# musevlt/muse-psfr

Measured on AMD Instinct MI355X. Metric: PSFs/sec (row x lambda) on 512^2 grid, 35 lambda, higher is better.
Workload: dtype f64 PSD->structure function, per-lambda OTF f32 -> split-fp16 MFMA (fp32 accumulate), f64 fit

## Files before the change

### muse_psfr_amd/csrc/fit_common.h

```cpp
#pragma once
#include <hip/hip_runtime.h>
#include "device_common.h"

namespace mpsfr {
namespace {

template <int CTRL, int ROW_MASK>
__device__ __forceinline__ float dpp_term(float v) {
    return __builtin_bit_cast(float, __builtin_amdgcn_update_dpp(
                                         0, __builtin_bit_cast(int, v), CTRL, ROW_MASK, 0xf, false));
}
template <int CTRL, int ROW_MASK>
__device__ __forceinline__ double dpp_term(double v) {
    const long long b = __builtin_bit_cast(long long, v);
    const unsigned lo = (unsigned)__builtin_amdgcn_update_dpp(0, (int)(b & 0xffffffffll), CTRL,
                                                              ROW_MASK, 0xf, false);
    const unsigned hi = (unsigned)__builtin_amdgcn_update_dpp(0, (int)(b >> 32), CTRL, ROW_MASK,
                                                              0xf, false);
    return __builtin_bit_cast(double, ((long long)hi << 32) | (long long)lo);
}
__device__ __forceinline__ float lane63(float x) {
    return __builtin_bit_cast(float, __builtin_amdgcn_readlane(__builtin_bit_cast(int, x), 63));
}
__device__ __forceinline__ double lane63(double x) {
    const long long b = __builtin_bit_cast(long long, x);
    const unsigned lo = (unsigned)__builtin_amdgcn_readlane((int)(b & 0xffffffffll), 63);
    const unsigned hi = (unsigned)__builtin_amdgcn_readlane((int)(b >> 32), 63);
    return __builtin_bit_cast(double, ((long long)hi << 32) | (long long)lo);
}
template <typename T>
__device__ __forceinline__ T wave_total(T v) {
    v += dpp_term<0xB1, 0xf>(v);
    v += dpp_term<0x4E, 0xf>(v);
    v += dpp_term<0x141, 0xf>(v);
    v += dpp_term<0x140, 0xf>(v);
    v += dpp_term<0x142, 0xf>(v);
    v += dpp_term<0x143, 0xf>(v);
    return lane63(v);
}

template <typename RE>
__device__ __forceinline__ RE fit_log(RE x);
template <>
__device__ __forceinline__ float fit_log<float>(float x) { return __logf(x); }
template <>
__device__ __forceinline__ double fit_log<double>(double x) { return log(x); }
template <typename RE>
__device__ __forceinline__ RE fit_exp(RE x);
template <>
__device__ __forceinline__ float fit_exp<float>(float x) { return __expf(x); }
template <>
__device__ __forceinline__ double fit_exp<double>(double x) { return exp(x); }

template <typename S>
__device__ __forceinline__ S fit_rcp(S x);
template <>
__device__ __forceinline__ float fit_rcp<float>(float x) { return __builtin_amdgcn_rcpf(x); }
template <>
__device__ __forceinline__ double fit_rcp<double>(double x) { return 1.0 / x; }
template <typename S>
__device__ __forceinline__ S fit_rsqrt(S x);
template <>
__device__ __forceinline__ float fit_rsqrt<float>(float x) { return __builtin_amdgcn_rsqf(x); }
template <>
__device__ __forceinline__ double fit_rsqrt<double>(double x) {
    double y = __builtin_amdgcn_rsq(x);
    const double h = 0.5 * x;
    y = fma(y, fma(-h * y, y, 0.5), y);
    y = fma(y, fma(-h * y, y, 0.5), y);
    return y;
}

__device__ __forceinline__ double lean_exp(double z) {
    z = fmax(z, -700.0);
    const double k = rint(z * 1.4426950408889634074);
    double r = fma(-k, 6.93147180369123816490e-01, z);
    r = fma(-k, 1.90821492927058770002e-10, r);
    double p = 1.0 / 3628800.0;
    p = fma(p, r, 1.0 / 362880.0);
    p = fma(p, r, 1.0 / 40320.0);
    p = fma(p, r, 1.0 / 5040.0);
    p = fma(p, r, 1.0 / 720.0);
    p = fma(p, r, 1.0 / 120.0);
    p = fma(p, r, 1.0 / 24.0);
    p = fma(p, r, 1.0 / 6.0);
    p = fma(p, r, 0.5);
    p = fma(p, r, 1.0);
    p = fma(p, r, 1.0);
    return ldexp(p, (int)k);
}
__device__ __forceinline__ double lean_log(double x) {
    const double l0 = (double)(__builtin_amdgcn_logf((float)x) * 0.69314718f);
    const double d = fma(x, lean_exp(-l0), -1.0);
    return l0 + d * fma(d, fma(d, 1.0 / 3.0, -0.5), 1.0);
}

template <typename RE>
__device__ __forceinline__ RE fit_exp2m1(RE eta);
template <>
__device__ __forceinline__ float fit_exp2m1<float>(float eta) {
    return __builtin_amdgcn_exp2f(eta) - 1.0f;
}
template <>
__device__ __forceinline__ double fit_exp2m1<double>(double eta) {
    return lean_exp(0.69314718055994530942 * eta) - 1.0;
}

template <typename RE>
__device__ __forceinline__ RE fit_log2(RE x);
template <>
__device__ __forceinline__ float fit_log2<float>(float x) { return __builtin_amdgcn_logf(x); }
template <>
__device__ __forceinline__ double fit_log2<double>(double x) { return log(x) * 1.4426950408889634074; }
template <typename RE>
__device__ __forceinline__ RE fit_exp2(RE x);
template <>
__device__ __forceinline__ float fit_exp2<float>(float x) { return __builtin_amdgcn_exp2f(x); }
template <>
__device__ __forceinline__ double fit_exp2<double>(double x) { return exp(x * 0.69314718055994530942); }

__device__ __forceinline__ double sgpr(double x) {
    const long long b = __builtin_bit_cast(long long, x);
    const unsigned lo = (unsigned)__builtin_amdgcn_readfirstlane((int)(b & 0xffffffffll));
    const unsigned hi = (unsigned)__builtin_amdgcn_readfirstlane((int)(b >> 32));
    return __builtin_bit_cast(double, ((long long)hi << 32) | (long long)lo);
}


constexpr double kFitIllCond = 100.0;
constexpr double kFitMaxE = 0.95;
#ifndef MPSFR_FIT_MAXIT
#define MPSFR_FIT_MAXIT 200
#endif
constexpr int kFitMaxIt = MPSFR_FIT_MAXIT;
constexpr double kFitMu0 = 1.0e-2, kFitMuMax = 1.0e15;

template <typename T, int NP>
struct FitNormEq {
    T a[NP * (NP + 1) / 2];
    T g[NP];
    T chi2;
};

template <int NP>
__host__ __device__ constexpr int fit_diag(int k) { return k * NP - k * (k - 1) / 2; }

template <int NP, typename S, typename T, bool ROW_FIRST = false>
__device__ __forceinline__ bool fit_chol(const FitNormEq<T, NP>& ne, S mu, S L[NP][NP], S Li[NP], S id[NP]) {
    bool ok = true;
#pragma unroll
    for (int i = 0; i < NP; ++i) {
        const S d = (S)ne.a[fit_diag<NP>(i)];
        ok = ok && (d > (S)0);
        id[i] = fit_rsqrt<S>(d);
    }
    {
        int k = 0;
#pragma unroll
        for (int i = 0; i < NP; ++i)
#pragma unroll
            for (int j = i; j < NP; ++j) {
                L[j][i] = ROW_FIRST ? (S)ne.a[k] * id[j] * id[i] : (S)ne.a[k] * id[i] * id[j];
                ++k;
            }
    }
#pragma unroll
    for (int j = 0; j < NP; ++j) {
        S s = (S)1 + mu;
#pragma unroll
        for (int q = 0; q < j; ++q) s -= L[j][q] * L[j][q];
        ok = ok && (s > (S)0);
        Li[j] = fit_rsqrt<S>(s);
        L[j][j] = s * Li[j];
#pragma unroll
        for (int i = j + 1; i < NP; ++i) {
            S t = L[i][j];
#pragma unroll
            for (int q = 0; q < j; ++q) t -= L[i][q] * L[j][q];
            L[i][j] = t * Li[j];
        }
    }
    return ok;
}

template <int NP, typename S, typename X>
__device__ __forceinline__ void fit_chol_solve(const S L[NP][NP], const S Li[NP], const S id[NP], const S b[NP],
                                               X* x) {
    S y[NP], z[NP];
#pragma unroll
    for (int i = 0; i < NP; ++i) {
        S t = b[i] * id[i];
#pragma unroll
        for (int q = 0; q < i; ++q) t -= L[i][q] * y[q];
        y[i] = t * Li[i];
    }
#pragma unroll
    for (int i = NP - 1; i >= 0; --i) {
        S t = y[i];
#pragma unroll
        for (int q = i + 1; q < NP; ++q) t -= L[q][i] * z[q];
        z[i] = t * Li[i];
    }
#pragma unroll
    for (int i = 0; i < NP; ++i) x[i] = (X)(z[i] * id[i]);
}

template <int NP, typename S, typename T, bool ROW_FIRST = false>
__device__ __forceinline__ bool fit_lm_solve(const FitNormEq<T, NP>& ne, S mu, S* x) {
    S L[NP][NP], Li[NP], id[NP], b[NP];
    if (!fit_chol<NP, S, T, ROW_FIRST>(ne, mu, L, Li, id)) return false;
#pragma unroll
    for (int i = 0; i < NP; ++i) b[i] = -(S)ne.g[i];
    fit_chol_solve<NP, S, S>(L, Li, id, b, x);
    return true;
}

template <int NP, typename T, bool ROW_FIRST = false>
__device__ __forceinline__ bool fit_spd_inverse(const FitNormEq<T, NP>& ne, double cov[NP][NP]) {
    T L[NP][NP], Li[NP], id[NP];
    if (!fit_chol<NP, T, T, ROW_FIRST>(ne, (T)0, L, Li, id)) return false;
#pragma unroll
    for (int c = 0; c < NP; ++c) {
        T b[NP];
        double x[NP];
#pragma unroll
        for (int k = 0; k < NP; ++k) b[k] = (k == c) ? (T)1 : (T)0;
        fit_chol_solve<NP, T, double>(L, Li, id, b, x);
#pragma unroll
        for (int k = 0; k < NP; ++k) cov[k][c] = x[k];
    }
    return true;
}

template <typename RE, bool ELL>
struct MoffatPar {
    RE I, p0, q0, n, gK, A, B, C, e1g2, e2g2, w2, nsq2, dKn;
    __device__ __forceinline__ MoffatPar(const RE* v, int ieta) {
        I = v[0]; p0 = v[1]; q0 = v[2];
        n = fit_rcp<RE>(v[ieta]);
        const RE s_ = fit_exp2m1<RE>(v[ieta]);
        const RE iw = fit_rcp<RE>(v[3]);
        const RE K = (RE)4 * s_ * iw * iw;
        if constexpr (ELL) {
            const RE e1 = v[4], e2 = v[5];
            const RE g2 = fit_rcp<RE>((RE)1 - e1 * e1 - e2 * e2);
            const RE g = fit_rsqrt<RE>((RE)1 - e1 * e1 - e2 * e2);
            gK = g * K;
            A = gK * ((RE)1 - e1); B = gK * e2; C = gK * ((RE)1 + e1);
            e1g2 = e1 * g2; e2g2 = e2 * g2;
        } else {
            gK = K; A = K; B = (RE)0; C = K; e1g2 = (RE)0; e2g2 = (RE)0;
        }
        w2 = (RE)2 * iw;
        nsq2 = n * n * (RE)0.69314718055994530942;
        dKn = (s_ + (RE)1) * (RE)0.69314718055994530942 * fit_rcp<RE>(s_);
    }
};

__device__ __forceinline__ bool fit_moment_start(float ms1, float ms2, float best, int rm, float* eta0, double* fw0) {
    const float bf = best, r2 = ((float)rm + 0.5f) * ((float)rm + 0.5f);
    if (!(rm >= 6 && ms1 > 0.f && best > 0.f)) return false;
    float t1 = 1.f, t2 = 1.f, nn = 2.5f, a2 = 1.f;
#pragma unroll 1
    for (int k = 0; k < 6; ++k) {
        float rho = (ms2 * t1) * __builtin_amdgcn_rcpf(bf * ms1 * t2);
        rho = fminf(fmaxf(rho, 0.05f), 0.47f);
        nn = (1.f - rho) * __builtin_amdgcn_rcpf(1.f - 2.f * rho);
        nn = fminf(fmaxf(nn, 1.1f), 15.f);
        a2 = ms1 * (nn - 1.f) * __builtin_amdgcn_rcpf(t1 * bf * 3.14159265f);
        const float lx = __builtin_amdgcn_logf(1.f + r2 * __builtin_amdgcn_rcpf(a2));
        t1 = 1.f - __builtin_amdgcn_exp2f((1.f - nn) * lx);
        t2 = 1.f - __builtin_amdgcn_exp2f((1.f - 2.f * nn) * lx);
    }
    *eta0 = __builtin_amdgcn_rcpf(nn);
    const float w = 2.f * __builtin_amdgcn_sqrtf(a2 * (__builtin_amdgcn_exp2f(*eta0) - 1.f));
    if (w == w) *fw0 = fmin(fmax((double)w, 1.5), (double)NS);
    return true;
}

}
}
```

### muse_psfr_amd/csrc/stamps.hip

```cpp
#include "device_common.h"
#include "conv_frames.h"
#include "fit_common.h"

namespace mpsfr {

namespace {

template <typename R>
__global__ void __launch_bounds__(256)
k_moffat_kernels(const double* __restrict__ gam, const double* __restrict__ alp,
                 R* __restrict__ out) {
    __shared__ double part[4];
    __shared__ double tot;
    const int k = blockIdx.x;
    const double g2 = gam[k] * gam[k], al = alp[k];
    double vals[(KS * KS + 255) / 256];
    double s = 0.0;
#pragma unroll
    for (int m = 0; m < (KS * KS + 255) / 256; ++m) {
        const int e = threadIdx.x + m * 256;
        double v = 0.0;
        if (e < KS * KS) {
            const int dy = e / KS - KS / 2, dx = e % KS - KS / 2;
            const double x1 = 1.0 + (double)(dx * dx + dy * dy) / g2;
            v = al == 2.0 ? 1.0 / (x1 * x1) : pow(x1, -al);
        }
        vals[m] = v;
        s += v;
    }
    s = wave_sum(s);
    if ((threadIdx.x & 63) == 0) part[threadIdx.x >> 6] = s;
    __syncthreads();
    if (threadIdx.x == 0) tot = (part[0] + part[1]) + (part[2] + part[3]);
    __syncthreads();
    const double inv = 1.0 / tot;
#pragma unroll
    for (int m = 0; m < (KS * KS + 255) / 256; ++m) {
        const int e = threadIdx.x + m * 256;
        if (e < KS * KS) out[(size_t)k * KS * KS + e] = (R)(vals[m] * inv);
    }
}

template <typename R>
struct Vec4;
template <>
struct Vec4<float> { using type = float4; };
template <>
struct Vec4<double> { using type = double4; };

template <typename R>
__global__ void __launch_bounds__(256)
k_conv(int nl, int tdiv, const R* __restrict__ pre, const R* __restrict__ ktt,
       const R* __restrict__ kmuse, double* __restrict__ fin) {
    constexpr int PH = NS + KS - 1;
    constexpr int PW = 84;
    constexpr int HK = KS / 2;
    constexpr int SW = 8;
    constexpr int LW = SW + KS - 1;
    constexpr int NSTRIP = NS * NS / SW;
    using V4 = typename Vec4<R>::type;
    extern __shared__ __align__(32) unsigned char smem[];
    R* img = reinterpret_cast<R*>(smem);
    const int l = blockIdx.x, task = blockIdx.y;
    const R* src = pre + ((size_t)task * nl + l) * NS * NS;
    for (int e = threadIdx.x; e < PH * PW; e += 256) {
        const int P = e / PW - HK, Q = e % PW - HK;
        img[e] = (P >= 0 && P < NS && Q >= 0 && Q < NS) ? (R)src[P * NS + Q] : (R)0;
    }
    static_assert(NSTRIP == 200 && NS == 40, "strip map assumes 40x40 stamps");
    const int wv = threadIdx.x >> 6, ln = threadIdx.x & 63;
    const bool active = ln < 50;
    const int i = 10 * wv + (active ? ln % 10 : 0), j0 = (active ? ln / 10 : 0) * SW;
    double acc[SW];
    for (int pass = 0; pass < 2; ++pass) {
        const R* __restrict__ kg = pass == 0 ? ktt + (size_t)(task / tdiv) * KS * KS
                                             : kmuse + (size_t)l * KS * KS;
        __syncthreads();
#pragma unroll
        for (int o = 0; o < SW; ++o) acc[o] = 0.0;
        for (int a = 0; a <= HK; ++a) {
            const V4* r1 = reinterpret_cast<const V4*>(
                __builtin_assume_aligned(img + (i - a + 2 * HK) * PW + j0, sizeof(V4)));
            const V4* r2 = reinterpret_cast<const V4*>(
                __builtin_assume_aligned(img + (i + a) * PW + j0, sizeof(V4)));
            R sv[LW];
#pragma unroll
            for (int c = 0; c < LW / 4; ++c) {
                const V4 q = r1[c];
                sv[4 * c] = q.x; sv[4 * c + 1] = q.y; sv[4 * c + 2] = q.z; sv[4 * c + 3] = q.w;
            }
            if (a < HK) {
#pragma unroll
                for (int c = 0; c < LW / 4; ++c) {
                    const V4 q = r2[c];
                    sv[4 * c] += q.x; sv[4 * c + 1] += q.y; sv[4 * c + 2] += q.z; sv[4 * c + 3] += q.w;
                }
            }
            R part[SW];
#pragma unroll
            for (int o = 0; o < SW; ++o) part[o] = (R)0;
            const R* __restrict__ krow = kg + a * KS;
#pragma unroll
            for (int b = 0; b < KS; ++b) {
                const R kv = krow[b];
#pragma unroll
                for (int o = 0; o < SW; ++o) part[o] += kv * sv[o - b + 2 * HK];
            }
#pragma unroll
            for (int o = 0; o < SW; ++o) acc[o] += (double)part[o];
        }
        __syncthreads();
        if (pass == 0 && active) {
#pragma unroll
            for (int o = 0; o < SW; ++o) img[(i + HK) * PW + j0 + HK + o] = (R)acc[o];
        }
    }
    if (active) {
        double* out = fin + ((size_t)task * nl + l) * NS * NS + i * NS + j0;
#pragma unroll
        for (int o = 0; o < SW; ++o) out[o] = acc[o];
    }
}

template <typename R, typename TF>
#ifndef MPSFR_CONV_WAVES
#define MPSFR_CONV_WAVES 4
#endif
__global__ void __launch_bounds__(256) __attribute__((amdgpu_waves_per_eu(sizeof(R) == 4 ? MPSFR_CONV_WAVES : 2)))
k_conv_fft(int nl, int tdiv, const R* __restrict__ pre, const cx<R>* __restrict__ khat_tt,
           const cx<R>* __restrict__ khat_muse, TF* __restrict__ fin) {
    extern __shared__ __align__(16) unsigned char conv_smem[];
    cx<R> (*F)[CFP] = reinterpret_cast<cx<R> (*)[CFP]>(conv_smem);
    cx<R> (*bufs)[CFB] = reinterpret_cast<cx<R> (*)[CFB]>(conv_smem + sizeof(cx<R>) * CF * CFP);
    const int l = blockIdx.x, task = blockIdx.y;
    const int slot = threadIdx.x >> 3, t = threadIdx.x & 7;
    Tw64<R> tw;
    tw.init(t);
    const R* src = pre + ((size_t)task * nl + l) * NS * NS;
    cx<R>* buf = bufs[slot];
    cx<R> x[8];
#pragma unroll
    for (int e = 0; e < 8; ++e) {
        const int c = t + 8 * e;
        const bool in = c < NS && slot < NS / 2;
        x[e] = {in ? src[2 * slot * NS + c] : (R)0, in ? src[(2 * slot + 1) * NS + c] : (R)0};
    }
    for (int pass = 0; pass < 2; ++pass) {
        const cx<R>* __restrict__ kh = pass == 0 ? khat_tt + (size_t)(task / tdiv) * (CFH + 1) * CF
                                                     : khat_muse + (size_t)l * (CFH + 1) * CF;
        cx<R> khv[8], khn[8];
#pragma unroll
        for (int e = 0; e < 8; ++e) {
            khv[e] = kh[slot * CF + t + 8 * e];
            khn[e] = slot == 0 ? kh[CFH * CF + t + 8 * e] : cx<R>{(R)0, (R)0};
        }
        __syncthreads();
        if (slot < NS / 2) cf_rows_forward(x, F, buf, tw, slot, t);
        __syncthreads();
        {
            cx<R> y[8];
            if (slot == 0) {
                const cx<R>* res = cf_col_forward(F, NS, buf, tw, slot, t);
#pragma unroll
                for (int e = 0; e < 8; ++e) {
                    cx<R> a0, a32;
                    cf_split0(res, t + 8 * e, a0, a32);
                    const cx<R> b0 = cmul(a0, khv[e]), b32 = cmul(a32, khn[e]);
                    y[e] = conjf<R>(cx<R>{b0.x - b32.y, b0.y + b32.x});
                }
                fft_sync<true>();
            } else {
                cx<R> xin[8], v[8];
#pragma unroll
                for (int e = 0; e < 8; ++e) {
                    const int r = t + 8 * e;
                    xin[e] = r < NS ? F[r][slot] : cx<R>{(R)0, (R)0};
                }
                fft_forward_regs_lastreg<R, CF, true>(xin, buf, buf, tw.w, t, v);
#pragma unroll
                for (int e = 0; e < 8; ++e) y[e] = conjf<R>(cmul(v[e], khv[e]));
                fft_sync<true>();
            }
            cx<R> r2[8];
            fft_forward_regs_lastreg<R, CF, true>(y, buf, buf, tw.w, t, r2);
#pragma unroll
            for (int e = 0; e < 8; ++e) {
                const int r = t + 8 * e;
                if (r >= KS / 2 && r < KS / 2 + NS) F[r][slot] = conjf<R>(r2[e]);
            }
        }
        __syncthreads();
        if (slot < NS / 2) {
            const int ra = KS / 2 + 2 * slot, rb = ra + 1;
            cx<R> z[8];
#pragma unroll
            for (int e = 0; e < 8; ++e) {
                const int k = t + 8 * e;
                const int kk = k <= CFH ? k : CF - k;
                cx<R> a, b;
                if (kk == 0) {
                    a = {F[ra][0].x, (R)0};
                    b = {F[rb][0].x, (R)0};
                } else if (kk == CFH) {
                    a = {F[ra][0].y, (R)0};
                    b = {F[rb][0].y, (R)0};
                } else {
                    a = F[ra][kk];
                    b = F[rb][kk];
                    if (k > CFH) { a = conjf<R>(a); b = conjf<R>(b); }
                }
                z[e] = {a.x - b.y, -(a.y + b.x)};
            }
            if (pass == 1) {
                cx<R> v[8];
                fft_forward_regs_lastreg<R, CF, true>(z, buf, buf, tw.w, t, v);
                TF* out = fin + ((size_t)task * nl + l) * NS * NS;
#pragma unroll
                for (int e = 0; e < 8; ++e) {
                    const int c = t + 8 * e;
                    if (c >= KS / 2 && c < KS / 2 + NS) {
                        const int i = 2 * slot, j = c - KS / 2;
                        out[i * NS + j] = (TF)v[e].x;
                        out[(i + 1) * NS + j] = (TF)(-v[e].y);
                    }
                }
            } else {
                const cx<R>* res = fft_forward_regs<R, CF, true>(z, buf, buf, tw.w, t);
#pragma unroll
                for (int e = 0; e < 8; ++e) {
                    const int c = t + 8 * e;
                    const cx<R> v = res[lds_out<CF, 8>(c < NS ? c + KS / 2 : 0)];
                    x[e] = c < NS ? cx<R>{v.x, -v.y} : cx<R>{(R)0, (R)0};
                }
            }
        }
    }
}

template <typename R>
__global__ void __launch_bounds__(256)
k_khat(const double* __restrict__ gam, const double* __restrict__ alp, cx<R>* __restrict__ khat) {
    extern __shared__ __align__(16) unsigned char conv_smem[];
    khat_body<R>(gam, alp, khat, conv_smem, (int)blockIdx.x);
}



typedef float f32x2 __attribute__((ext_vector_type(2)));

template <typename RE>
struct NormAcc {
    RE a[15], g[5], chi2;
    __device__ __forceinline__ void zero() {
#pragma unroll
        for (int k = 0; k < 15; ++k) a[k] = (RE)0;
#pragma unroll
        for (int k = 0; k < 5; ++k) g[k] = (RE)0;
        chi2 = (RE)0;
    }
    __device__ __forceinline__ void add(const RE* J, RE r) {
        chi2 += r * r;
        int k = 0;
#pragma unroll
        for (int x = 0; x < 5; ++x) {
            g[x] += J[x] * r;
#pragma unroll
            for (int y = x; y < 5; ++y) a[k++] += J[x] * J[y];
        }
    }
    template <typename F>
    __device__ __forceinline__ void totals(FitNormEq<RE, 5>& ne, F total) const {
        ne.chi2 = total(chi2);
#pragma unroll
        for (int k = 0; k < 15; ++k) ne.a[k] = total(a[k]);
#pragma unroll
        for (int k = 0; k < 5; ++k) ne.g[k] = total(g[k]);
    }
};
template <>
struct NormAcc<float> {
    f32x2 r0a, r0b, r0c;
    f32x2 r1b, r1c;
    f32x2 r2b, r2c;
    f32x2 r3c, r4c;
    float a11, a33, chi2;
    __device__ __forceinline__ void zero() {
        const f32x2 z = {0.f, 0.f};
        r0a = r0b = r0c = r1b = r1c = r2b = r2c = r3c = r4c = z;
        a11 = a33 = chi2 = 0.f;
    }
    __device__ __forceinline__ void add(const float* J, float r) {
        const f32x2 p01 = {J[0], J[1]}, p23 = {J[2], J[3]}, p4r = {J[4], r};
        const f32x2 s0 = {J[0], J[0]}, s1 = {J[1], J[1]}, s2 = {J[2], J[2]}, s3 = {J[3], J[3]},
                    s4 = {J[4], J[4]};
        r0a += s0 * p01; r0b += s0 * p23; r0c += s0 * p4r;
        r1b += s1 * p23; r1c += s1 * p4r;
        r2b += s2 * p23; r2c += s2 * p4r;
        r3c += s3 * p4r;
        r4c += s4 * p4r;
        a11 += J[1] * J[1];
        a33 += J[3] * J[3];
        chi2 += r * r;
    }
    template <typename F>
    __device__ __forceinline__ void totals(FitNormEq<float, 5>& ne, F total) const {
        ne.chi2 = total(chi2);
        const float a[15] = {r0a.x, r0a.y, r0b.x, r0b.y, r0c.x, a11, r1b.x, r1b.y, r1c.x,
                             r2b.x, r2b.y, r2c.x, a33, r3c.x, r4c.x};
        const float g[5] = {r0c.y, r1c.y, r2c.y, r3c.y, r4c.y};
#pragma unroll
        for (int k = 0; k < 15; ++k) ne.a[k] = total(a[k]);
#pragma unroll
        for (int k = 0; k < 5; ++k) ne.g[k] = total(g[k]);
    }
};

template <typename RE>
__device__ __forceinline__ void moffat_accumulate(const RE* pix, int lane, const RE* v,
                                                  FitNormEq<RE, 5>& ne) {
    constexpr int NPX = NS * NS / 64;
    NormAcc<RE> acc;
    acc.zero();
    const RE n = fit_rcp<RE>(v[4]);
    const RE s_ = fit_exp2m1<RE>(v[4]);
    const RE i3 = fit_rcp<RE>(v[3]);
    const RE K = (RE)4 * s_ * i3 * i3;
    const RE dKn = (s_ + (RE)1) * (RE)0.69314718055994530942 * fit_rcp<RE>(s_);
    const RE I = v[0], p0 = v[1], q0 = v[2];
    const RE nsq2 = n * n * (RE)0.69314718055994530942;
    const RE c12 = (RE)2 * n * K, c3 = c12 * i3, c4 = n * K * dKn;
    const RE lrf = (RE)(lane >> 3) - p0, lcf = (RE)(lane & 7) - q0;
    const RE* pl = pix + (lane >> 3) * NS + (lane & 7);
    static_assert(NPX == 25 && NS == 40, "5 x 5 blocks of 8 x 8 pixels");
#pragma unroll 1
    for (int mo = 0; mo < 5; ++mo) {
        const RE dp = (RE)(8 * mo) + lrf, dp2 = dp * dp;
#pragma unroll
        for (int mi = 0; mi < 5; ++mi) {
        const RE dq = (RE)(8 * mi) + lcf;
        const RE u = dq * dq + dp2;
        const RE gg = (RE)1 + u * K;
        const RE lg2 = fit_log2<RE>(gg);
        const RE e = fit_exp2<RE>(-n * lg2);
        const RE mo_ = I * e;
        const RE r = mo_ - pl[mo * 8 * NS + mi * 8];
        const RE t = mo_ * fit_rcp<RE>(gg);
        const RE tu = t * u, tc = t * c12;
        RE J[5];
        J[0] = e;
        J[1] = tc * dp;
        J[2] = tc * dq;
        J[3] = tu * c3;
        J[4] = mo_ * (nsq2 * lg2) - tu * c4;
        acc.add(J, r);
        }
    }
    acc.totals(ne, [](RE x) { return wave_total(x); });
}

#ifndef MPSFR_FIT_PAIRS
#define MPSFR_FIT_PAIRS 1
#endif
__device__ __forceinline__ void moffat_accumulate_pairs(const float* pix, int lane, const float* v,
                                                        FitNormEq<float, 5>& ne) {
    f32x2 A[15], G[5], C = {0.f, 0.f};
#pragma unroll
    for (int k = 0; k < 15; ++k) A[k] = f32x2{0.f, 0.f};
#pragma unroll
    for (int k = 0; k < 5; ++k) G[k] = f32x2{0.f, 0.f};
    const float n = fit_rcp<float>(v[4]);
    const float s_ = fit_exp2m1<float>(v[4]);
    const float i3 = fit_rcp<float>(v[3]);
    const float K = 4.f * s_ * i3 * i3;
    const float dKn = (s_ + 1.f) * 0.69314718f * fit_rcp<float>(s_);
    const float I = v[0], p0 = v[1], q0 = v[2];
    const float nsq2 = n * n * 0.69314718f;
    const float c12 = 2.f * n * K, c3 = c12 * i3, c4 = n * K * dKn;
    const f32x2 K2 = {K, K}, I2 = {I, I}, nn2 = {-n, -n}, nsq22 = {nsq2, nsq2}, c122 = {c12, c12},
                c32 = {c3, c3}, c42 = {c4, c4}, one2 = {1.f, 1.f};
    const float lrf = (float)(lane >> 3) - p0, lcf = (float)(lane & 7) - q0;
    const float* pl = pix + (lane >> 3) * NS + (lane & 7);
    auto pair = [&](f32x2 u, f32x2 dpv, f32x2 dqv, f32x2 px, bool last) {
        const f32x2 gg = u * K2 + one2;
        const f32x2 lg2 = {fit_log2<float>(gg.x), fit_log2<float>(gg.y)};
        const f32x2 arg = lg2 * nn2;
        f32x2 e = {fit_exp2<float>(arg.x), fit_exp2<float>(arg.y)};
        if (last) e.y = 0.f;
        const f32x2 m = e * I2;
        const f32x2 r = m - px;
        const f32x2 rg = {fit_rcp<float>(gg.x), fit_rcp<float>(gg.y)};
        const f32x2 t = m * rg;
        const f32x2 tu = t * u, tc = t * c122;
        f32x2 J[5];
        J[0] = e;
        J[1] = tc * dpv;
        J[2] = tc * dqv;
        J[3] = tu * c32;
        J[4] = m * (lg2 * nsq22) - tu * c42;
        C += r * r;
        int k = 0;
#pragma unroll
        for (int x = 0; x < 5; ++x) {
            G[x] += J[x] * r;
#pragma unroll
            for (int y = x; y < 5; ++y) A[k++] += J[x] * J[y];
        }
    };
    const f32x2 dqa = {lcf, 8.f + lcf}, dqb = {16.f + lcf, 24.f + lcf};
    const f32x2 dqa2 = dqa * dqa, dqb2 = dqb * dqb;
    const float dq4 = 32.f + lcf, dq4s = dq4 * dq4;
#pragma unroll 1
    for (int mo = 0; mo < 5; ++mo) {
        const float dp = (float)(8 * mo) + lrf, dp2 = dp * dp;
        const f32x2 dpv = {dp, dp}, dp2v = {dp2, dp2};
        const float* row = pl + mo * 8 * NS;
        pair(dqa2 + dp2v, dpv, dqa, f32x2{row[0], row[8]}, false);
        pair(dqb2 + dp2v, dpv, dqb, f32x2{row[16], row[24]}, false);
    }
    {
        const f32x2 dq4v = {dq4, dq4}, dq4sv = {dq4s, dq4s};
        const f32x2 dpa = {lrf, 8.f + lrf}, dpb = {16.f + lrf, 24.f + lrf};
        const float dp4 = 32.f + lrf;
        pair(dpa * dpa + dq4sv, dpa, dq4v, f32x2{pl[32], pl[8 * NS + 32]}, false);
        pair(dpb * dpb + dq4sv, dpb, dq4v, f32x2{pl[16 * NS + 32], pl[24 * NS + 32]}, false);
        pair(f32x2{dp4 * dp4 + dq4s, 0.f}, f32x2{dp4, 0.f}, dq4v, f32x2{pl[32 * NS + 32], 0.f}, true);
    }
    ne.chi2 = wave_total(C.x + C.y);
#pragma unroll
    for (int k = 0; k < 15; ++k) ne.a[k] = wave_total(A[k].x + A[k].y);
#pragma unroll
    for (int k = 0; k < 5; ++k) ne.g[k] = wave_total(G[k].x + G[k].y);
}

template <typename RE>
__device__ __forceinline__ void lm_accumulate(const RE* pix, int lane, const RE* v, FitNormEq<RE, 5>& ne) {
    if constexpr (sizeof(RE) == 4 && MPSFR_FIT_PAIRS) moffat_accumulate_pairs(pix, lane, v, ne);
    else moffat_accumulate<RE>(pix, lane, v, ne);
}

template <typename RE, typename DT>
__device__ __forceinline__ RE moffat_chi2(const DT* pix, int lane, const double* va) {
    const RE I = (RE)va[0], p0 = (RE)va[1], q0 = (RE)va[2], n = (RE)va[4];
    const RE K = (RE)(1.0 / (va[3] * va[3]));
    RE c[5] = {(RE)0, (RE)0, (RE)0, (RE)0, (RE)0};
    const RE lrf = (RE)(lane >> 3) - p0, lcf = (RE)(lane & 7) - q0;
    const DT* pl = pix + (lane >> 3) * NS + (lane & 7);
#pragma unroll 1
    for (int mo = 0; mo < 5; ++mo) {
        const RE dp = (RE)(8 * mo) + lrf;
#pragma unroll
        for (int mi = 0; mi < 5; ++mi) {
            const RE dq = (RE)(8 * mi) + lcf;
            const RE r = I * fit_exp<RE>(-n * fit_log<RE>((RE)1 + (dp * dp + dq * dq) * K)) -
                         (RE)pl[mo * 8 * NS + mi * 8];
            c[mi] += r * r;
        }
    }
    return wave_total(((c[0] + c[1]) + (c[2] + c[3])) + c[4]);
}


template <typename TS>
__device__ __forceinline__ void moffat_gradient(const TS* __restrict__ src, int lane,
                                                const double* v, double* gout, double* chi2out) {
    const double n = sgpr(1.0 / v[4]);
    const double s = lean_exp(0.69314718055994530942 * v[4]) - 1.0;
    const double K = sgpr(4.0 * s / (v[3] * v[3]));
    const float dKn = (float)sgpr((s + 1.0) * 0.69314718055994530942 / s);
    const float nsq = (float)(n * n);
    const double I = sgpr(v[0]), p0 = sgpr(v[1]), q0 = sgpr(v[2]);
    const float i3 = (float)sgpr(1.0 / v[3]), nf = (float)n, K2 = 2.0f * (float)K, Kf = (float)K;
    float g[5] = {0.f, 0.f, 0.f, 0.f, 0.f}, c2sum = 0.f;
    const double lrd = (double)(lane >> 3) - p0, lcd = (double)(lane & 7) - q0;
    const TS* pl = src + (lane >> 3) * NS + (lane & 7);
#pragma unroll 1
    for (int mo = 0; mo < 5; ++mo) {
        const double dp = (double)(8 * mo) + lrd, dp2 = dp * dp;
#pragma unroll
        for (int mi = 0; mi < 5; ++mi) {
        const double dq = (double)(8 * mi) + lcd;
        const double u = fma(dq, dq, dp2);
        const double gg = 1.0 + u * K;
        const double lg = lean_log(gg);
        const double e = lean_exp(-n * lg);
        const double mo_ = I * e;
        const float r = (float)(mo_ - (double)pl[mo * 8 * NS + mi * 8]);
        c2sum += r * r;
        const float mof = (float)mo_, uf = (float)u;
        const float cm = mof * nf * __builtin_amdgcn_rcpf((float)gg);
        const float c2 = cm * K2 * r;
        g[0] += (float)e * r;
        g[1] += c2 * (float)dp;
        g[2] += c2 * (float)dq;
        g[3] += c2 * uf * i3;
        g[4] += (nsq * mof * (float)lg - cm * uf * Kf * dKn) * r;
        }
    }
#pragma unroll
    for (int k = 0; k < 5; ++k) gout[k] = wave_total((double)g[k]);
    *chi2out = (double)wave_total(c2sum);
}

#ifndef MPSFR_POLISH_TOL
#define MPSFR_POLISH_TOL 1.0e-4
#endif
#ifndef MPSFR_FIT_WAVES
#define MPSFR_FIT_WAVES 3
#endif
template <typename RE>
constexpr int fit_min_waves() { return sizeof(RE) == 4 ? MPSFR_FIT_WAVES : 2; }

#ifndef MPSFR_FIT_MOMENT_START
#define MPSFR_FIT_MOMENT_START 1
#endif
struct SumArgs {
    int nwg, ntask, nl, accumulate;
    double* sum;
};

#ifndef MPSFR_FIT_WG
#define MPSFR_FIT_WG 1
#endif
template <typename RE, typename TS>
__global__ void __launch_bounds__(64 * MPSFR_FIT_WG) __attribute__((amdgpu_waves_per_eu(fit_min_waves<RE>())))
k_fit(int nstamp, const TS* __restrict__ stamps, double* __restrict__ fit, double polish_tol, SumArgs sa) {
    constexpr int NPX = NS * NS / 64;
    static_assert(NPX * 64 == NS * NS, "the lane map assumes 1600 pixels");
    using S = RE;
    const int lane = threadIdx.x & 63;
    if ((int)blockIdx.x < sa.nwg) {
        const size_t per = (size_t)sa.nl * NS * NS;
        const size_t e = ((size_t)blockIdx.x * MPSFR_FIT_WG + (threadIdx.x >> 6)) * 64 + lane;
        if (e >= per) return;
        double acc = 0.0;
        int t = 0;
        for (; t + 8 <= sa.ntask; t += 8) {
            TS v[8];
#pragma unroll
            for (int k = 0; k < 8; ++k) v[k] = stamps[(size_t)(t + k) * per + e];
#pragma unroll
            for (int k = 0; k < 8; ++k) acc += (double)v[k];
        }
        for (; t < sa.ntask; ++t) acc += (double)stamps[(size_t)t * per + e];
        sa.sum[e] = sa.accumulate ? sa.sum[e] + acc : acc;
        return;
    }
    const int st = ((int)blockIdx.x - sa.nwg) * MPSFR_FIT_WG + (threadIdx.x >> 6);
    if (st >= nstamp) return;
    const TS* src = stamps + (size_t)st * NS * NS;
    __shared__ RE spix[MPSFR_FIT_WG][NS * NS];
    RE* sp = spix[threadIdx.x >> 6];
    TS best = (TS)-3.0e38;
    int besto = 0;
#pragma unroll
    for (int m = 0; m < NPX; ++m) {
        const int o = lane + m * 64;
        const TS d = src[o];
        sp[o] = (RE)d;
        if (d > best) { best = d; besto = o; }
    }
#pragma unroll
    for (int o = 32; o > 0; o >>= 1) {
        const TS ob = __shfl_xor(best, o, 64);
        const int oo = __shfl_xor(besto, o, 64);
        if (ob > best || (ob == best && oo < besto)) { best = ob; besto = oo; }
    }
    const int p0i = besto / NS, q0i = besto % NS;
    const int rm = min(min(p0i, NS - 1 - p0i), min(q0i, NS - 1 - q0i));
    const float abest = fabsf((float)best);
    const bool amp_ok = abest >= 0x1p-40f && abest <= 0x1p40f;
    int cnt = 0;
    const TS half = (TS)0.5 * best;
    float ms1 = 0.f, ms2 = 0.f;
    {
        const float r2 = ((float)rm + 0.5f) * ((float)rm + 0.5f);
        const float lrf = (float)((lane >> 3) - p0i), lcf = (float)((lane & 7) - q0i);
        const RE* pl = sp + (lane >> 3) * NS + (lane & 7);
#pragma unroll
        for (int mo = 0; mo < 5; ++mo) {
            const float dp = (float)(8 * mo) + lrf, dp2 = dp * dp;
#pragma unroll
            for (int mi = 0; mi < 5; ++mi) {
                const float dq = (float)(8 * mi) + lcf;
                const float d = (float)pl[mo * 8 * NS + mi * 8];
                cnt += (TS)pl[mo * 8 * NS + mi * 8] > half ? 1 : 0;
                const float din = fmaf(dq, dq, dp2) <= r2 ? d : 0.f;
                ms1 += din;
                ms2 = fmaf(din, din, ms2);
            }
        }
    }
#pragma unroll
    for (int o = 32; o > 0; o >>= 1) cnt += __shfl_xor(cnt, o, 64);
    ms1 = wave_total(ms1);
    ms2 = wave_total(ms2);
    double fw0 = 2.0 * sqrt((double)cnt / kPi);
    fw0 = fmin(fmax(fw0, 1.5), (double)NS);
    float eta0 = 0.4f;
    if (MPSFR_FIT_MOMENT_START) fit_moment_start(ms1, ms2, (float)best, rm, &eta0, &fw0);
    S v[5] = {(S)best, (S)p0i, (S)q0i, (S)fw0, (S)eta0};
#ifndef MPSFR_FIT_TOL_F32
#define MPSFR_FIT_TOL_F32 1.0e-3
#endif
    const S tol = sizeof(RE) == 4 ? (S)MPSFR_FIT_TOL_F32 : (S)1.0e-10;
    FitNormEq<RE, 5> ne;
    lm_accumulate<RE>(sp, lane, v, ne);
    S mu = (S)kFitMu0, nu = (S)2;
    const S mu_max = (S)kFitMuMax;
    int it = 0, status = amp_ok ? 1 : 2;
    const int maxit = amp_ok ? kFitMaxIt : 0;
    while (it < maxit) {
        ++it;
        S dx[5];
        if (!fit_lm_solve<5, S, RE, true>(ne, mu, dx)) {
            mu *= nu;
            nu *= (S)2;
            if (mu > mu_max) { status = 2; break; }
            continue;
        }
        if (v[4] + dx[4] < (S)0.2 * v[4]) {
            const S sc = (S)-0.8 * v[4] * fit_rcp<S>(dx[4]);
#pragma unroll
            for (int k = 0; k < 5; ++k) dx[k] *= sc;
        }
        S vn[5], rel = (S)0;
#pragma unroll
        for (int k = 0; k < 5; ++k) {
            vn[k] = v[k] + dx[k];
            rel = fmax(rel, fabs(dx[k]) * fit_rcp<S>(fabs(vn[k]) + (S)1.0e-30));
        }
        const bool inside = vn[3] > (S)1.0e-3 && vn[4] > (S)1.0e-3 && vn[4] < (S)1.0e2;
        if (inside && rel < tol) {
#pragma unroll
            for (int k = 0; k < 5; ++k) v[k] = vn[k];
            status = 0;
            break;
        }
        FitNormEq<RE, 5> nn;
        S rho = (S)-1;
        if (inside) {
            lm_accumulate<RE>(sp, lane, vn, nn);
            S pred = (S)0;
#pragma unroll
            for (int k = 0; k < 5; ++k)
                pred += dx[k] * (mu * (S)ne.a[fit_diag<5>(k)] * dx[k] - (S)ne.g[k]);
            rho = ((S)ne.chi2 - (S)nn.chi2) * fit_rcp<S>(pred);
        }
        if (rho > (S)0) {
#pragma unroll
            for (int k = 0; k < 5; ++k) v[k] = vn[k];
            ne = nn;
            if (v[4] < (S)1.5e-3) { status = 0; break; }
            const S c = (S)2 * rho - (S)1;
            mu = fmax(mu * fmax((S)(1.0 / 3.0), (S)1 - c * c * c), (S)1.0e-14);
            nu = (S)2;
        } else {
            mu *= nu;
            nu *= (S)2;
            if (mu > mu_max) { status = 0; break; }
        }
    }
    double vd[5];
#pragma unroll
    for (int k = 0; k < 5; ++k) vd[k] = (double)v[k];
    double polish_chi2 = -1.0;
    if constexpr (sizeof(RE) == 4) {
        FitNormEq<double, 5> np;
#pragma unroll
        for (int k = 0; k < 15; ++k) np.a[k] = (double)ne.a[k];
        np.chi2 = -1.0;
#ifndef MPSFR_POLISH_MAX
#define MPSFR_POLISH_MAX 8
#endif
        for (int pz = 0; pz < MPSFR_POLISH_MAX && status != 2; ++pz) {
            moffat_gradient(src, lane, vd, np.g, &np.chi2);
            double dx[5];
            if (!fit_lm_solve<5, double, double, true>(np, 1.0e-10, dx)) break;
            float rel = 0.f;
#pragma unroll
            for (int k = 0; k < 5; ++k)
                rel = fmaxf(rel, fabsf((float)dx[k]) *
                                     __builtin_amdgcn_rcpf(fabsf((float)(vd[k] + dx[k])) + 1.0e-30f));
            const bool inside = vd[3] + dx[3] > 1.0e-3 && vd[4] + dx[4] > 1.0e-3 &&
                                vd[4] + dx[4] < 1.0e2 && rel < 0.1f;
            if (!inside) break;
#pragma unroll
            for (int k = 0; k < 5; ++k) vd[k] += dx[k];
            ++it;
            polish_chi2 = rel < 1.0e-3f ? np.chi2 : -1.0;
            if (rel < (float)polish_tol) break;
        }
    }
    const double n = 1.0 / vd[4];
    const double p2 = exp2(1.0 / n), s2 = p2 - 1.0, sq = sqrt(s2);
    const double al = fabs(vd[3]) / (2.0 * sq);
    const double va[5] = {vd[0], vd[1], vd[2], al, n};
    double chi2 = polish_chi2;
    if (chi2 < 0.0) chi2 = (double)moffat_chi2<RE>(sp, lane, va);
    if (lane == 0) {
        double* o = fit + (size_t)st * NFIT;
        o[0] = vd[0]; o[1] = vd[1]; o[2] = vd[2]; o[3] = al; o[4] = n;
        o[5] = fabs(vd[3]);
        o[6] = chi2;
        o[7] = (double)it;
        double cov[5][5];
        const double dof = (double)(NS * NS - 5);
        if (fit_spd_inverse<5, RE, true>(ne, cov)) {
            const double s = chi2 / dof;
            o[8] = sqrt(fmax(cov[0][0] * s, 0.0));
            o[9] = sqrt(fmax(cov[1][1] * s, 0.0));
            o[10] = sqrt(fmax(cov[2][2] * s, 0.0));
            const double aw = 1.0 / (2.0 * sq);
            const double an = -al * p2 * 0.69314718055994530942 / (2.0 * s2);
            const double var = aw * aw * cov[3][3] + 2.0 * aw * an * cov[3][4] + an * an * cov[4][4];
            o[11] = sqrt(fmax(var * s, 0.0));
            o[12] = n * n * sqrt(fmax(cov[4][4] * s, 0.0));
            o[13] = sqrt(fmax(cov[3][3] * s, 0.0));
            if (n * n * sqrt(fmax(cov[4][4], 0.0)) * fabs(vd[0]) >= kFitIllCond) status |= 4;
        } else {
            for (int k = 0; k < 6; ++k) o[8 + k] = 0.0;
            if (status == 0) status = 2;
        }
        bool finite_row = isfinite(chi2);
#pragma unroll
        for (int k = 0; k < 5; ++k) finite_row = finite_row && isfinite(vd[k]);
        if ((status & 3) == 0 && !finite_row) status = (status & 4) | 2;
        if ((status & 3) == 0 && vd[4] > 90.0) status = (status & 4) | 1;
        o[14] = (double)status;
        o[15] = vd[0] * kPi * al * al / (n - 1.0);
    }
}

template <typename TF>
__global__ void __launch_bounds__(256) k_stamp_sum(int ntask, int nl, const TF* __restrict__ fin,
                                                   double* __restrict__ sum, int accumulate) {
    __shared__ double part[4][64];
    const int wave = threadIdx.x >> 6, lane = threadIdx.x & 63;
    const size_t e = (size_t)blockIdx.x * 64 + lane;
    const size_t per = (size_t)nl * NS * NS;
    double s = 0.0;
    if (e < per) {
        int t = wave;
        for (; t + 28 < ntask; t += 32) {
            TF v[8];
#pragma unroll
            for (int k = 0; k < 8; ++k) v[k] = fin[(size_t)(t + 4 * k) * per + e];
#pragma unroll
            for (int k = 0; k < 8; ++k) s += (double)v[k];
        }
        for (; t < ntask; t += 4) s += (double)fin[(size_t)t * per + e];
    }
    part[wave][lane] = s;
    __syncthreads();
    if (wave == 0 && e < per) {
        const double tot = (part[0][lane] + part[1][lane]) + (part[2][lane] + part[3][lane]);
        sum[e] = accumulate ? sum[e] + tot : tot;
    }
}

constexpr int kBlobCopyThreads = 1024, kBlobCopyPer = 4;
__global__ void __launch_bounds__(kBlobCopyThreads) k_param_copy(uint4* __restrict__ dst, const uint4* __restrict__ src, int n16,
                                                                  unsigned long long* flag, unsigned long long seq) {
    for (int base = 0; base < n16; base += kBlobCopyThreads * kBlobCopyPer) {
        uint4 v[kBlobCopyPer];
#pragma unroll
        for (int q = 0; q < kBlobCopyPer; ++q) {
            const int i = base + q * kBlobCopyThreads + (int)threadIdx.x;
            if (i < n16) v[q] = src[i];
        }
#pragma unroll
        for (int q = 0; q < kBlobCopyPer; ++q) {
            const int i = base + q * kBlobCopyThreads + (int)threadIdx.x;
            if (i < n16) dst[i] = v[q];
        }
    }
    if (flag != nullptr) {
        __syncthreads();
        if (threadIdx.x == 0) {
            __threadfence_system();
            __hip_atomic_store(flag, seq, __ATOMIC_RELEASE, __HIP_MEMORY_SCOPE_SYSTEM);
        }
    }
}

}

void launch_param_copy(hipStream_t s, void* d_dst, const void* h_src_pinned, size_t bytes,
                       unsigned long long* h_flag_pinned, unsigned long long seq) {
    const int n16 = (int)(bytes / 16);
    if (n16 <= 0) return;
    const int nthr = n16 >= kBlobCopyThreads ? kBlobCopyThreads : (n16 + 63) / 64 * 64;
    hipLaunchKernelGGL(k_param_copy, dim3(1), dim3(nthr), 0, s, (uint4*)d_dst, (const uint4*)h_src_pinned, n16,
                       h_flag_pinned, seq);
}

void launch_moffat_kernels(hipStream_t s, int nker, const double* d_gamma, const double* d_alpha,
                           void* d_out, bool f64) {
    if (nker <= 0) return;
    if (f64)
        hipLaunchKernelGGL(k_moffat_kernels<double>, dim3(nker), dim3(256), 0, s, d_gamma, d_alpha,
                           (double*)d_out);
    else
        hipLaunchKernelGGL(k_moffat_kernels<float>, dim3(nker), dim3(256), 0, s, d_gamma, d_alpha,
                           (float*)d_out);
}

void launch_conv(hipStream_t s, int ntask, int nl, const void* d_pre, const void* d_ktt,
                 const void* d_kmuse, double* d_fin, bool f64, int tdiv) {
    dim3 grid(nl, ntask);
    constexpr int PH = NS + KS - 1, PW = 84;
    if (f64) {
        const size_t sm = (size_t)(PH * PW) * sizeof(double);
        hipLaunchKernelGGL(k_conv<double>, grid, dim3(256), sm, s, nl, tdiv, (const double*)d_pre,
                           (const double*)d_ktt,
                           (const double*)d_kmuse, d_fin);
    } else {
        const size_t sm = (size_t)(PH * PW) * sizeof(float);
        hipLaunchKernelGGL(k_conv<float>, grid, dim3(256), sm, s, nl, tdiv, (const float*)d_pre,
                           (const float*)d_ktt,
                           (const float*)d_kmuse, d_fin);
    }
}

void launch_khat(hipStream_t s, int nker, const double* d_gamma, const double* d_alpha,
                 void* d_khat, bool f64) {
    if (nker <= 0) return;
    if (f64) {
        allow_smem(k_khat<double>, conv_smem_bytes<double>(true));
        hipLaunchKernelGGL(k_khat<double>, dim3(nker), dim3(256), conv_smem_bytes<double>(true), s, d_gamma,
                           d_alpha, (cx<double>*)d_khat);
    } else {
        hipLaunchKernelGGL(k_khat<float>, dim3(nker), dim3(256), conv_smem_bytes<float>(true), s, d_gamma,
                           d_alpha, (cx<float>*)d_khat);
    }
}

void launch_conv_fft(hipStream_t s, int ntask, int nl, const void* d_pre, const void* d_khat_tt,
                     const void* d_khat_muse, void* d_fin, bool fin_f32, bool f64, int tdiv) {
    const dim3 grid(nl, ntask);
    if (f64) {
        allow_smem((k_conv_fft<double, double>), conv_smem_bytes<double>(false));
        hipLaunchKernelGGL((k_conv_fft<double, double>), grid, dim3(256), conv_smem_bytes<double>(false), s, nl, tdiv,
                           (const double*)d_pre, (const cx<double>*)d_khat_tt, (const cx<double>*)d_khat_muse,
                           (double*)d_fin);
    } else if (fin_f32) {
        hipLaunchKernelGGL((k_conv_fft<float, float>), grid, dim3(256), conv_smem_bytes<float>(false), s, nl, tdiv,
                           (const float*)d_pre, (const cx<float>*)d_khat_tt, (const cx<float>*)d_khat_muse,
                           (float*)d_fin);
    } else {
        hipLaunchKernelGGL((k_conv_fft<float, double>), grid, dim3(256), conv_smem_bytes<float>(false), s, nl, tdiv,
                           (const float*)d_pre, (const cx<float>*)d_khat_tt, (const cx<float>*)d_khat_muse,
                           (double*)d_fin);
    }
}

void launch_fit(hipStream_t s, int nstamp, const void* d_stamps, bool stamps_f32, double* d_fit,
                bool f64, int sum_ntask, int sum_nl, double* d_sum, int sum_accumulate) {
    if (nstamp <= 0) return;
    SumArgs sa = {0, sum_ntask, sum_nl, sum_accumulate, d_sum};
    if (d_sum != nullptr && sum_ntask > 0) {
        const size_t per = (size_t)sum_nl * NS * NS;
        sa.nwg = (int)((per + 64 * MPSFR_FIT_WG - 1) / (64 * MPSFR_FIT_WG));
    }
    const dim3 grid(sa.nwg + (nstamp + MPSFR_FIT_WG - 1) / MPSFR_FIT_WG), blk(64 * MPSFR_FIT_WG);
#ifndef MPSFR_FIT_F64_LM
#define MPSFR_FIT_F64_LM 0
#endif
    if (f64 && MPSFR_FIT_F64_LM)
        hipLaunchKernelGGL((k_fit<double, double>), grid, blk, 0, s, nstamp,
                           (const double*)d_stamps, d_fit, 0.0, sa);
    else if (stamps_f32)
// ... 22 lines not shown
```

Before: 19.57 million.

## Batch wave reductions via transposed DPP tree and parallelize covariance columns per lane

Replaces per-value wave_total reductions of the 21 normal-equation terms, the gradient and the moment sums with a batched reduction. Each DPP step halves the number of live values by having lanes keep alternate partial sums, and permlane16/32 swaps finish the cross-row stages. The argmax shuffle-xor loop becomes DPP plus permlane steps. The covariance inverse now solves one column per lane instead of all columns serially on lane 0. Polish also reads from the shared-memory stamp copy when types match. The cost is more intricate lane bookkeeping, and the inline asm needs the permlane swap instructions to exist on the target.

```diff
diff --git a/muse_psfr_amd/csrc/fit_common.h b/muse_psfr_amd/csrc/fit_common.h
--- a/muse_psfr_amd/csrc/fit_common.h
+++ b/muse_psfr_amd/csrc/fit_common.h
@@ -37,6 +37,98 @@
     v += dpp_term<0x142, 0xf>(v);
     v += dpp_term<0x143, 0xf>(v);
     return lane63(v);
+}
+
+template <int CTRL>
+__device__ __forceinline__ int dpp_pull(int own) {
+    return __builtin_amdgcn_update_dpp(own, own, CTRL, 0xf, 0xf, false);
+}
+template <int CTRL>
+__device__ __forceinline__ float dpp_pull(float own) {
+    return __builtin_bit_cast(float, dpp_pull<CTRL>(__builtin_bit_cast(int, own)));
+}
+template <int CTRL>
+__device__ __forceinline__ double dpp_pull(double own) {
+    const long long b = __builtin_bit_cast(long long, own);
+    const unsigned lo = (unsigned)dpp_pull<CTRL>((int)(b & 0xffffffffll));
+    const unsigned hi = (unsigned)dpp_pull<CTRL>((int)(b >> 32));
+    return __builtin_bit_cast(double, ((long long)hi << 32) | (long long)lo);
+}
+__device__ __forceinline__ float lane_pick(bool second, float a, float b) { return second ? b : a; }
+__device__ __forceinline__ double lane_pick(bool second, double a, double b) { return second ? b : a; }
+__device__ __forceinline__ void rows_swap16(unsigned& a, unsigned& b) {
+    asm("s_nop 1\n\tv_permlane16_swap_b32 %0, %1" : "+v"(a), "+v"(b));
+}
+__device__ __forceinline__ void rows_swap32(unsigned& a, unsigned& b) {
+    asm("s_nop 1\n\tv_permlane32_swap_b32 %0, %1" : "+v"(a), "+v"(b));
+}
+template <bool HALVES>
+__device__ __forceinline__ void rows_swap(float& a, float& b) {
+    unsigned x = __builtin_bit_cast(unsigned, a), y = __builtin_bit_cast(unsigned, b);
+    if constexpr (HALVES) rows_swap32(x, y);
+    else rows_swap16(x, y);
+    a = __builtin_bit_cast(float, x);
+    b = __builtin_bit_cast(float, y);
+}
+template <bool HALVES>
+__device__ __forceinline__ void rows_swap(double& a, double& b) {
+    const unsigned long long x = __builtin_bit_cast(unsigned long long, a), y = __builtin_bit_cast(unsigned long long, b);
+    unsigned xl = (unsigned)x, xh = (unsigned)(x >> 32), yl = (unsigned)y, yh = (unsigned)(y >> 32);
+    if constexpr (HALVES) { rows_swap32(xl, yl); rows_swap32(xh, yh); }
+    else { rows_swap16(xl, yl); rows_swap16(xh, yh); }
+    a = __builtin_bit_cast(double, ((unsigned long long)xh << 32) | xl);
+    b = __builtin_bit_cast(double, ((unsigned long long)yh << 32) | yl);
+}
+template <int LANE>
+__device__ __forceinline__ float lane_value(float x) {
+    return __builtin_bit_cast(float, __builtin_amdgcn_readlane(__builtin_bit_cast(int, x), LANE));
+}
+template <int LANE>
+__device__ __forceinline__ double lane_value(double x) {
+    const long long b = __builtin_bit_cast(long long, x);
+    const unsigned lo = (unsigned)__builtin_amdgcn_readlane((int)(b & 0xffffffffll), LANE);
+    const unsigned hi = (unsigned)__builtin_amdgcn_readlane((int)(b >> 32), LANE);
+    return __builtin_bit_cast(double, ((long long)hi << 32) | (long long)lo);
+}
+template <int CTRL, int N, typename T>
+__device__ __forceinline__ void wave_totals_step(const T (&in)[N], T (&out)[(N + 1) / 2], bool second) {
+#pragma unroll
+    for (int j = 0; j < N / 2; ++j) {
+        const T a = in[2 * j] + dpp_term<CTRL, 0xf>(in[2 * j]);
+        const T b = in[2 * j + 1] + dpp_term<CTRL, 0xf>(in[2 * j + 1]);
+        out[j] = lane_pick(second, a, b);
+    }
+    if constexpr (N % 2 == 1) out[N / 2] = in[N - 1] + dpp_term<CTRL, 0xf>(in[N - 1]);
+}
+__host__ __device__ constexpr int wave_totals_lane(int k) {
+    const int b3 = (k >> 3) & 1, b2 = ((k >> 2) & 1) ^ b3, b1 = ((k >> 1) & 1) ^ b2, b0 = (k & 1) ^ b2;
+    return b3 * 8 + b2 * 4 + b1 * 2 + b0;
+}
+template <int K, int N, typename T>
+__device__ __forceinline__ void wave_totals_read(T (&v)[N], T r) {
+    if constexpr (K < N) {
+        v[K] = lane_value<(K >> 4) * 16 + wave_totals_lane(K & 15)>(r);
+        if constexpr (((K + 1) & 15) != 0) wave_totals_read<K + 1, N, T>(v, r);
+    }
+}
+template <int N, typename T>
+__device__ __forceinline__ void wave_totals(T (&v)[N], int lane) {
+    static_assert(N >= 1 && N <= 32, "one or two registers of 16 values");
+    constexpr int N1 = (N + 1) / 2, N2 = (N1 + 1) / 2, N3 = (N2 + 1) / 2, N4 = (N3 + 1) / 2;
+    T s1[N1], s2[N2], s3[N3], s4[N4];
+    const int b2 = (lane >> 2) & 1;
+    wave_totals_step<0xB1>(v, s1, ((lane ^ b2) & 1) != 0);
+    wave_totals_step<0x4E>(s1, s2, (((lane >> 1) ^ b2) & 1) != 0);
+    wave_totals_step<0x141>(s2, s3, (((lane >> 3) ^ b2) & 1) != 0);
+    wave_totals_step<0x140>(s3, s4, (lane & 8) != 0);
+    static_assert(N4 == (N + 15) / 16, "16 values per register");
+    T a = s4[0], b = s4[N4 - 1];
+    rows_swap<false>(a, b);
+    T p = b + a, q = p;
+    rows_swap<true>(p, q);
+    const T t = q + p;
+    wave_totals_read<0, N, T>(v, t);
+    if constexpr (N > 16) wave_totals_read<16, N, T>(v, t);
 }
 
 template <typename RE>
@@ -229,6 +321,20 @@
 #pragma unroll
         for (int k = 0; k < NP; ++k) cov[k][c] = x[k];
     }
+    return true;
+}
+
+template <int NP, typename T, bool ROW_FIRST = false>
+__device__ __forceinline__ bool fit_spd_inverse_column(const FitNormEq<T, NP>& ne, int lane, double x[NP]) {
+    T L[NP][NP], Li[NP], id[NP], b[NP];
+    if (!fit_chol<NP, T, T, ROW_FIRST>(ne, (T)0, L, Li, id)) {
+#pragma unroll
+        for (int k = 0; k < NP; ++k) x[k] = 0.0;
+        return false;
+    }
+#pragma unroll
+    for (int k = 0; k < NP; ++k) b[k] = (k == lane) ? (T)1 : (T)0;
+    fit_chol_solve<NP, T, double>(L, Li, id, b, x);
     return true;
 }
 
diff --git a/muse_psfr_amd/csrc/stamps.hip b/muse_psfr_amd/csrc/stamps.hip
--- a/muse_psfr_amd/csrc/stamps.hip
+++ b/muse_psfr_amd/csrc/stamps.hip
@@ -1,6 +1,7 @@
 #include "device_common.h"
 #include "conv_frames.h"
 #include "fit_common.h"
+#include <type_traits>
 
 namespace mpsfr {
 
@@ -249,6 +250,16 @@
 typedef float f32x2 __attribute__((ext_vector_type(2)));
 
 template <typename RE>
+__device__ __forceinline__ void norm_totals(RE (&t)[21], FitNormEq<RE, 5>& ne, int lane) {
+    wave_totals(t, lane);
+    ne.chi2 = t[0];
+#pragma unroll
+    for (int k = 0; k < 15; ++k) ne.a[k] = t[1 + k];
+#pragma unroll
+    for (int k = 0; k < 5; ++k) ne.g[k] = t[16 + k];
+}
+
+template <typename RE>
 struct NormAcc {
     RE a[15], g[5], chi2;
     __device__ __forceinline__ void zero() {
@@ -268,13 +279,14 @@
             for (int y = x; y < 5; ++y) a[k++] += J[x] * J[y];
         }
     }
-    template <typename F>
-    __device__ __forceinline__ void totals(FitNormEq<RE, 5>& ne, F total) const {
-        ne.chi2 = total(chi2);
-#pragma unroll
-        for (int k = 0; k < 15; ++k) ne.a[k] = total(a[k]);
-#pragma unroll
-        for (int k = 0; k < 5; ++k) ne.g[k] = total(g[k]);
+    __device__ __forceinline__ void totals(FitNormEq<RE, 5>& ne, int lane) const {
+        RE t[21];
+        t[0] = chi2;
+#pragma unroll
+        for (int k = 0; k < 15; ++k) t[1 + k] = a[k];
+#pragma unroll
+        for (int k = 0; k < 5; ++k) t[16 + k] = g[k];
+        norm_totals(t, ne, lane);
     }
 };
 template <>
@@ -302,16 +314,10 @@
         a33 += J[3] * J[3];
         chi2 += r * r;
     }
-    template <typename F>
-    __device__ __forceinline__ void totals(FitNormEq<float, 5>& ne, F total) const {
-        ne.chi2 = total(chi2);
-        const float a[15] = {r0a.x, r0a.y, r0b.x, r0b.y, r0c.x, a11, r1b.x, r1b.y, r1c.x,
-                             r2b.x, r2b.y, r2c.x, a33, r3c.x, r4c.x};
-        const float g[5] = {r0c.y, r1c.y, r2c.y, r3c.y, r4c.y};
-#pragma unroll
-        for (int k = 0; k < 15; ++k) ne.a[k] = total(a[k]);
-#pragma unroll
-        for (int k = 0; k < 5; ++k) ne.g[k] = total(g[k]);
+    __device__ __forceinline__ void totals(FitNormEq<float, 5>& ne, int lane) const {
+        float t[21] = {chi2, r0a.x, r0a.y, r0b.x, r0b.y, r0c.x, a11, r1b.x, r1b.y, r1c.x,
+                       r2b.x, r2b.y, r2c.x, a33, r3c.x, r4c.x, r0c.y, r1c.y, r2c.y, r3c.y, r4c.y};
+        norm_totals(t, ne, lane);
     }
 };
 
@@ -355,7 +361,7 @@
         acc.add(J, r);
         }
     }
-    acc.totals(ne, [](RE x) { return wave_total(x); });
+    acc.totals(ne, lane);
 }
 
 #ifndef MPSFR_FIT_PAIRS
@@ -425,11 +431,13 @@
         pair(dpb * dpb + dq4sv, dpb, dq4v, f32x2{pl[16 * NS + 32], pl[24 * NS + 32]}, false);
         pair(f32x2{dp4 * dp4 + dq4s, 0.f}, f32x2{dp4, 0.f}, dq4v, f32x2{pl[32 * NS + 32], 0.f}, true);
     }
-    ne.chi2 = wave_total(C.x + C.y);
-#pragma unroll
-    for (int k = 0; k < 15; ++k) ne.a[k] = wave_total(A[k].x + A[k].y);
-#pragma unroll
-    for (int k = 0; k < 5; ++k) ne.g[k] = wave_total(G[k].x + G[k].y);
+    float t[21];
+    t[0] = C.x + C.y;
+#pragma unroll
+    for (int k = 0; k < 15; ++k) t[1 + k] = A[k].x + A[k].y;
+#pragma unroll
+    for (int k = 0; k < 5; ++k) t[16 + k] = G[k].x + G[k].y;
+    norm_totals(t, ne, lane);
 }
 
 template <typename RE>
@@ -462,7 +470,7 @@
 
 template <typename TS>
 __device__ __forceinline__ void moffat_gradient(const TS* __restrict__ src, int lane,
-                                                const double* v, double* gout, double* chi2out) {
+                                                const double* v, double (&gout)[5], double* chi2out) {
     const double n = sgpr(1.0 / v[4]);
     const double s = lean_exp(0.69314718055994530942 * v[4]) - 1.0;
     const double K = sgpr(4.0 * s / (v[3] * v[3]));
@@ -497,7 +505,8 @@
         }
     }
 #pragma unroll
-    for (int k = 0; k < 5; ++k) gout[k] = wave_total((double)g[k]);
+    for (int k = 0; k < 5; ++k) gout[k] = (double)g[k];
+    wave_totals(gout, lane);
     *chi2out = (double)wave_total(c2sum);
 }
 
@@ -521,6 +530,24 @@
 #ifndef MPSFR_FIT_WG
 #define MPSFR_FIT_WG 1
 #endif
+template <int CTRL, typename TS>
+__device__ __forceinline__ void fit_argmax_step(TS& best, int& besto) {
+    const TS ob = dpp_pull<CTRL>(best);
+    const int oo = dpp_pull<CTRL>(besto);
+    if (ob > best || (ob == best && oo < besto)) { best = ob; besto = oo; }
+}
+template <bool HALVES, typename TS>
+__device__ __forceinline__ void fit_argmax_rows(TS& best, int& besto) {
+    TS b0 = best, b1 = best;
+    float o0 = __builtin_bit_cast(float, besto), o1 = o0;
+    rows_swap<HALVES>(b0, b1);
+    rows_swap<HALVES>(o0, o1);
+    const int i0 = __builtin_bit_cast(int, o0), i1 = __builtin_bit_cast(int, o1);
+    const bool second = b1 > b0 || (b1 == b0 && i1 < i0);
+    best = second ? b1 : b0;
+    besto = second ? i1 : i0;
+}
+
 template <typename RE, typename TS>
 __global__ void __launch_bounds__(64 * MPSFR_FIT_WG) __attribute__((amdgpu_waves_per_eu(fit_min_waves<RE>())))
 k_fit(int nstamp, const TS* __restrict__ stamps, double* __restrict__ fit, double polish_tol, SumArgs sa) {
@@ -559,12 +586,12 @@
         sp[o] = (RE)d;
         if (d > best) { best = d; besto = o; }
     }
-#pragma unroll
-    for (int o = 32; o > 0; o >>= 1) {
-        const TS ob = __shfl_xor(best, o, 64);
-        const int oo = __shfl_xor(besto, o, 64);
-        if (ob > best || (ob == best && oo < besto)) { best = ob; besto = oo; }
-    }
+    fit_argmax_step<0xB1>(best, besto);
+    fit_argmax_step<0x4E>(best, besto);
+    fit_argmax_step<0x141>(best, besto);
+    fit_argmax_step<0x140>(best, besto);
+    fit_argmax_rows<false>(best, besto);
+    fit_argmax_rows<true>(best, besto);
     const int p0i = besto / NS, q0i = besto % NS;
     const int rm = min(min(p0i, NS - 1 - p0i), min(q0i, NS - 1 - q0i));
     const float abest = fabsf((float)best);
@@ -590,11 +617,11 @@
             }
         }
     }
-#pragma unroll
-    for (int o = 32; o > 0; o >>= 1) cnt += __shfl_xor(cnt, o, 64);
-    ms1 = wave_total(ms1);
-    ms2 = wave_total(ms2);
-    double fw0 = 2.0 * sqrt((double)cnt / kPi);
+    float ms[3] = {ms1, ms2, (float)cnt};
+    wave_totals(ms, lane);
+    ms1 = ms[0];
+    ms2 = ms[1];
+    double fw0 = 2.0 * sqrt((double)ms[2] / kPi);
     fw0 = fmin(fmax(fw0, 1.5), (double)NS);
     float eta0 = 0.4f;
     if (MPSFR_FIT_MOMENT_START) fit_moment_start(ms1, ms2, (float)best, rm, &eta0, &fw0);
@@ -673,7 +700,8 @@
 #define MPSFR_POLISH_MAX 8
 #endif
         for (int pz = 0; pz < MPSFR_POLISH_MAX && status != 2; ++pz) {
-            moffat_gradient(src, lane, vd, np.g, &np.chi2);
+            if constexpr (std::is_same<TS, RE>::value) moffat_gradient(sp, lane, vd, np.g, &np.chi2);
+            else moffat_gradient(src, lane, vd, np.g, &np.chi2);
             double dx[5];
             if (!fit_lm_solve<5, double, double, true>(np, 1.0e-10, dx)) break;
             float rel = 0.f;
@@ -697,26 +725,29 @@
     const double va[5] = {vd[0], vd[1], vd[2], al, n};
     double chi2 = polish_chi2;
     if (chi2 < 0.0) chi2 = (double)moffat_chi2<RE>(sp, lane, va);
+    double colx[5];
+    const bool spd = fit_spd_inverse_column<5, RE, true>(ne, lane, colx);
+    const double cov00 = lane_value<0>(colx[0]), cov11 = lane_value<1>(colx[1]), cov22 = lane_value<2>(colx[2]),
+                 cov33 = lane_value<3>(colx[3]), cov34 = lane_value<4>(colx[3]), cov44 = lane_value<4>(colx[4]);
     if (lane == 0) {
         double* o = fit + (size_t)st * NFIT;
         o[0] = vd[0]; o[1] = vd[1]; o[2] = vd[2]; o[3] = al; o[4] = n;
         o[5] = fabs(vd[3]);
         o[6] = chi2;
         o[7] = (double)it;
-        double cov[5][5];
         const double dof = (double)(NS * NS - 5);
-        if (fit_spd_inverse<5, RE, true>(ne, cov)) {
+        if (spd) {
             const double s = chi2 / dof;
-            o[8] = sqrt(fmax(cov[0][0] * s, 0.0));
-            o[9] = sqrt(fmax(cov[1][1] * s, 0.0));
-            o[10] = sqrt(fmax(cov[2][2] * s, 0.0));
+            o[8] = sqrt(fmax(cov00 * s, 0.0));
+            o[9] = sqrt(fmax(cov11 * s, 0.0));
+            o[10] = sqrt(fmax(cov22 * s, 0.0));
             const double aw = 1.0 / (2.0 * sq);
             const double an = -al * p2 * 0.69314718055994530942 / (2.0 * s2);
-            const double var = aw * aw * cov[3][3] + 2.0 * aw * an * cov[3][4] + an * an * cov[4][4];
+            const double var = aw * aw * cov33 + 2.0 * aw * an * cov34 + an * an * cov44;
             o[11] = sqrt(fmax(var * s, 0.0));
-            o[12] = n * n * sqrt(fmax(cov[4][4] * s, 0.0));
-            o[13] = sqrt(fmax(cov[3][3] * s, 0.0));
-            if (n * n * sqrt(fmax(cov[4][4], 0.0)) * fabs(vd[0]) >= kFitIllCond) status |= 4;
+            o[12] = n * n * sqrt(fmax(cov44 * s, 0.0));
+            o[13] = sqrt(fmax(cov33 * s, 0.0));
+            if (n * n * sqrt(fmax(cov44, 0.0)) * fabs(vd[0]) >= kFitIllCond) status |= 4;
         } else {
             for (int k = 0; k < 6; ++k) o[8 + k] = 0.0;
             if (status == 0) status = 2;
```

After: 19.89 million, median of 6. 1.02x the previous value.
